# swook/EVE

Hardware: AMD Instinct MI355X
Metric: train-step frames/sec, 128x128 eye patches T=30 (higher is better)
Workload: dtype bf16; 1 GPU; BASELINE configs[1]: EyeNet training (configs/eye_net.json: ResNet-18-IN + GRU-128, angular + pupil L1 losses, clip 5.0, Adam wd 0.005), 128x128 patches, fwd+bwd+clip+Adam; global_batch=32, batch_per_gpu=32, seq_len=30, parallelism=dp1

## Files before the change

eve_amd/csrc/conv_igemm.hip:

```cpp
#include <limits.h>
#include <stdio.h>
#include <stdlib.h>

#include <initializer_list>
#include <type_traits>
#include "common.h"

namespace eve {

struct GatherParams {
    int N, IH, IW, Cin;
    int OH, OW, Cout;
    int KH, KW;
    int o_mul, k_mul, off, div;
    int K;
    uint32_t M;
    FastDiv fd_ohw, fd_ow, fd_cin, fd_kw, fd_oh;
};

template <typename T>
__device__ __forceinline__ uint4 prologue_vec(uint4 q, const float* __restrict__ ssp, int act) {
    constexpr int VEC = Elem<T>::VEC;
    float f[VEC];
    Elem<T>::unpack(q, f);
// ... 478 lines not shown
}

template <typename T>
static void launch_dma_one(const GatherParams& p, const TapPlan& tp, const void* src, const void* w,
                           const float* bias, int epi_act, void* out, uint32_t src_bytes, uint32_t w_bytes,
                           hipStream_t s) {
    const T* a = (const T*)src; const T* b = (const T*)w; T* o = (T*)out;
    const int big = g_cfg.conv_tile_big;
    if (p.Cout > 64 && big && p.M >= 256 * 256) {
        const uint32_t tiles = ((p.M + 255) / 256) * ((p.Cout + 127) / 128);
        EVE_LAUNCH("igemm_dma_kernel<T, 4, 2>", (igemm_dma_kernel<T, 4, 2>), dim3(tiles), dim3(512), 0, s, p, a, b, bias, epi_act, o,
                           src_bytes, w_bytes, tp);
    } else if (p.Cout > 64) {
        const uint32_t tiles = ((p.M + 127) / 128) * ((p.Cout + 127) / 128);
        EVE_LAUNCH("igemm_dma_kernel<T, 2, 2>", (igemm_dma_kernel<T, 2, 2>), dim3(tiles), dim3(256), 0, s, p, a, b, bias, epi_act, o,
                           src_bytes, w_bytes, tp);
    } else {
        const uint32_t tiles = (p.M + 255) / 256;
        EVE_LAUNCH("igemm_dma_kernel<T, 4, 1>", (igemm_dma_kernel<T, 4, 1>), dim3(tiles), dim3(256), 0, s, p, a, b, bias, epi_act, o,
                           src_bytes, w_bytes, tp);
    }
}

template <typename HT>
static bool launch_halo(const GatherParams& p, const void* src, const void* w, const float* bias, int epi_act,
                        void* out, hipStream_t s) {
    if (!g_cfg.conv_halo) return false;
    const bool fwd = p.k_mul == 1 && p.off == -1, bwd = p.k_mul == -1 && p.off == 1;
    if (p.KH != 3 || p.KW != 3 || p.div != 1 || p.o_mul != 1 || !(fwd || bwd) || p.OH != p.IH || p.OW != p.IW) return false;
    const int W = p.IW, H = p.IH;
    if (p.Cin % 32 || W > 128 || (W & (W - 1)) || W < 4) return false;
    HaloParams h;
    h.N = p.N; h.H = H; h.W = W; h.Cin = p.Cin; h.Cout = p.Cout;
    const int ws64 = g_cfg.conv_ws64;
    if (ws64 && H == W && (W == 32 || W == 64) && p.Cin == 64 && p.Cout == 64 && ((epi_act & ~0xff) == 0) &&
        ((epi_act & 0xff) == EVE_ACT_NONE || (epi_act & 0xff) == EVE_ACT_RELU) && (unsigned long long)p.N * W * W * 128ull < (1ull << 31)) {
        Ws64Params q;
        q.N = p.N; q.flip = bwd ? 1 : 0; q.x_bytes = (uint32_t)((unsigned long long)p.N * W * W * 128ull); q.w_bytes = 64u * 576u * 2u;
        const uint32_t T64 = (uint32_t)(W * W / 512) * (uint32_t)p.N;
        if (W == 32)
            launch(EVE_KERNEL_H(HT, conv3x3_ws64_kernel, 32), dim3(T64 < 256u ? T64 : 256u), dim3(512), (size_t)Ws64Geom<32>::LDS, s, q,
                   (const HT*)src, (const HT*)w, bias, epi_act, (HT*)out);
        else
            launch(EVE_KERNEL_H(HT, conv3x3_ws64_kernel, 64), dim3(T64 < 256u ? T64 : 256u), dim3(512), (size_t)Ws64Geom<64>::LDS, s, q,
                   (const HT*)src, (const HT*)w, bias, epi_act, (HT*)out);
        return true;
    }
    const int wg8 = g_cfg.conv_wg8;
    const int wg8_min_tiles = g_cfg.conv_wg8_min_tiles;
    if (wg8 && H == W && p.Cin % 64 == 0 && ((epi_act & ~0xff) == 0) &&
        ((epi_act & 0xff) == EVE_ACT_NONE || (epi_act & 0xff) == EVE_ACT_RELU)) {
        const unsigned long long xb8 = (unsigned long long)p.N * H * W * p.Cin * 2, wb8 = (unsigned long long)p.Cout * p.K * 2;
        Wg8Params g;
        g.N = p.N; g.Cin = p.Cin; g.Cout = p.Cout; g.flip = bwd ? 1 : 0; g.K = p.K; g.x_bytes = (uint32_t)xb8; g.w_bytes = (uint32_t)wb8; g.s2_py = 0;
        auto wg8_tile = [&](auto kernel, auto geom, uint32_t units) {
            using G8 = decltype(geom);
            g.tiles_n = (uint32_t)(p.Cout / G8::COUT_T);
            const uint32_t tiles8 = (units + G8::TI - 1) / G8::TI * g.tiles_n;
            if ((int)tiles8 < wg8_min_tiles) return false;
            launch(kernel, dim3(tiles8), dim3(512), G8::LDS, s, g, (const HT*)src, (const HT*)w, bias, epi_act, (HT*)out);
            return true;
        };
        const uint32_t imgs = (uint32_t)p.N;
        if (xb8 < (1ull << 31) && wb8 < (1ull << 31)) {
            if (wg8 != 3 && W == 16 && p.Cout % 128 == 0 && p.Cout % 256 != 0 &&
                wg8_tile(EVE_KERNEL_H(HT, conv3x3_wg8_kernel, 4, 2, 16), Wg8Geom<4, 2, 16>{}, imgs)) return true;
            if (W == 16 && p.Cout % 256 == 0 && wg8_tile(EVE_KERNEL_H(HT, conv3x3_wg8_kernel, 2, 4, 16), Wg8Geom<2, 4, 16>{}, imgs)) return true;
            if (W == 8 && p.Cout % 256 == 0 && wg8_tile(EVE_KERNEL_H(HT, conv3x3_wg8_kernel, 2, 4, 8), Wg8Geom<2, 4, 8>{}, imgs)) return true;
            if (W == 4 && p.Cout % 256 == 0 && wg8_tile(EVE_KERNEL_H(HT, conv3x3_wg8_kernel, 2, 4, 4), Wg8Geom<2, 4, 4>{}, imgs)) return true;
            if (W == 32 && p.Cout % 128 == 0 &&
                wg8_tile(EVE_KERNEL_H(HT, conv3x3_wg8_kernel, 4, 2, 32, 9, 2), Wg8Geom<4, 2, 32, 2>{}, 2u * imgs)) return true;
        }
    }
    const bool narrow = p.Cout <= 64;
    const int BMp = narrow ? 256 : 128;
    const int rows = BMp / W;
    if (rows < 1) return false;
    if (rows <= H) { h.TI = 1; h.TH = rows; h.bands = (H + rows - 1) / rows; }
    else { if (rows % H) return false; h.TI = rows / H; h.TH = H; h.bands = 1; }
    const int HP = h.TI * (h.TH + 2) * (W + 2);
    h.a_pieces = (HP * 4 + 255) / 256;
    if (h.a_pieces > 7) return false;
    const unsigned long long xb = (unsigned long long)p.N * H * W * p.Cin * 2, wb = (unsigned long long)p.Cout * p.K * 2;
    if (xb >= (1ull << 31) || wb >= (1ull << 31)) return false;
    h.flip = bwd ? 1 : 0; h.K = p.K; h.x_bytes = (uint32_t)xb; h.w_bytes = (uint32_t)wb;
    h.tiles_m = h.TI == 1 ? (uint32_t)p.N * h.bands : (uint32_t)((p.N + h.TI - 1) / h.TI);
    h.tiles_n = narrow ? 1 : (p.Cout + 127) / 128;
    h.fd_w2 = make_fastdiv(W + 2); h.fd_hpi = make_fastdiv((h.TH + 2) * (W + 2)); h.fd_w = make_fastdiv(W); h.fd_th = make_fastdiv(h.TH);
    const size_t lds = 2 * (size_t)h.a_pieces * 4096 + 4 * (narrow ? 4096 : 8192);
    const int persist = g_cfg.halo_persist;
    const uint32_t tiles = h.tiles_m * h.tiles_n;
    if (persist && tiles > 512 && p.Cin <= 64 && p.Cout % 8 == 0 && (epi_act == EVE_ACT_NONE || epi_act == EVE_ACT_RELU)) {
        const size_t plds = lds + (bias ? (size_t)h.tiles_n * (narrow ? 64 : 128) * 4 : 0);
        if (narrow)
            launch(EVE_KERNEL_H(HT, conv3x3_halo_pkernel, 4, 1), dim3(512), dim3(256), plds, s, h, (const HT*)src, (const HT*)w, bias, epi_act, (HT*)out);
        else
            launch(EVE_KERNEL_H(HT, conv3x3_halo_pkernel, 2, 2), dim3(512), dim3(256), plds, s, h, (const HT*)src, (const HT*)w, bias, epi_act, (HT*)out);
        return true;
    }
    if (narrow)
        launch(EVE_KERNEL_H(HT, conv3x3_halo_kernel, 4, 1), dim3(tiles), dim3(256), lds, s, h, (const HT*)src, (const HT*)w, bias, epi_act, (HT*)out);
    else
        launch(EVE_KERNEL_H(HT, conv3x3_halo_kernel, 2, 2), dim3(tiles), dim3(256), lds, s, h, (const HT*)src, (const HT*)w, bias, epi_act, (HT*)out);
    return true;
}

template <typename T>
// ... 216 lines not shown
                wgrad_split(p, tk, tc, lds_bytes(64, 256, mode), splits, rows);
                if (mode == 1)      tr_tile(EVE_WGRAD_TR(T, 1, 4, 1, 4), tk, tc);
                else if (mode == 2) {
                    if (p.Cout <= 16)      tr_tile(EVE_WGRAD_TR(T, 1, 4, 2, 1), tk, tc);
                    else if (p.Cout <= 32) tr_tile(EVE_WGRAD_TR(T, 1, 4, 2, 2), tk, tc);
                    else                   tr_tile(EVE_WGRAD_TR(T, 1, 4, 2, 4), tk, tc);
                }
                else                tr_tile(EVE_WGRAD_TR(T, 1, 4, 0, 4), tk, tc);
            }
            return db ? 1 : 0;
        }
    }
    }
    const bool wide = p.Cout > 64;
    const uint32_t bco = wide ? 128 : 64;
    const uint32_t tk = (p.K + 127) / 128, tc = (p.Cout + bco - 1) / bco;
    uint32_t want = (1024 + tk * tc - 1) / (tk * tc);
    uint32_t max_splits = (p.M + 255) / 256;
    uint32_t splits = want < 1 ? 1 : (want > max_splits ? max_splits : want);
    if (splits < 1) splits = 1;
    if (splits > 65535) splits = 65535;
    uint32_t rows = (p.M + splits - 1) / splits;
    rows = (rows + 63) / 64 * 64;
    splits = (p.M + rows - 1) / rows;
    dim3 grid(tk, tc, splits), block(256);
    const T* a = (const T*)x; const T* b = (const T*)dy;
    if (wide) {
        if (ss) EVE_LAUNCH("wgrad_kernel<T, 4, true>", (wgrad_kernel<T, 4, true>), grid, block, 0, s, p, a, b, ss, pro_act, dw, rows);
        else    EVE_LAUNCH("wgrad_kernel<T, 4, false>", (wgrad_kernel<T, 4, false>), grid, block, 0, s, p, a, b, ss, pro_act, dw, rows);
    } else {
        if (ss) EVE_LAUNCH("wgrad_kernel<T, 2, true>", (wgrad_kernel<T, 2, true>), grid, block, 0, s, p, a, b, ss, pro_act, dw, rows);
        else    EVE_LAUNCH("wgrad_kernel<T, 2, false>", (wgrad_kernel<T, 2, false>), grid, block, 0, s, p, a, b, ss, pro_act, dw, rows);
    }
    return 0;
}

template <typename HT>
static bool launch_s2_fwd_wg8(const eve_conv_desc* d, const void* x, const void* w, const float* bias, int epi_act, void* y, hipStream_t s) {
    const int on = g_cfg.conv_wg8, min_tiles = g_cfg.conv_wg8_s2_min_tiles;
    const int W = d->OW;
    if (!on || d->KH != 3 || d->KW != 3 || d->stride != 2 || d->pad != 1 || d->OH != W || d->IH != 2 * W || d->IW != 2 * W ||
        !(W == 16 || W == 8 || W == 4) || d->Cin % 64 || (epi_act & ~0xff) ||
        !((epi_act & 0xff) == EVE_ACT_NONE || (epi_act & 0xff) == EVE_ACT_RELU))
        return false;
    const int cout_t = W == 16 ? 128 : 256;
    if (d->Cout % cout_t) return false;
    const unsigned long long xb = (unsigned long long)d->N * 4 * W * W * d->Cin * 2, wb = (unsigned long long)d->Cout * 9 * d->Cin * 2;
    if (xb >= (1ull << 31) || wb >= (1ull << 31)) return false;
    const int ti = W == 16 ? 2 : (W == 8 ? 4 : 16);
    const uint32_t tiles = (uint32_t)((d->N + ti - 1) / ti) * (uint32_t)(d->Cout / cout_t);
    if ((int)tiles < min_tiles) return false;
    Wg8Params g;
    g.N = d->N; g.Cin = d->Cin; g.Cout = d->Cout; g.flip = 0; g.K = 9 * d->Cin; g.x_bytes = (uint32_t)xb; g.w_bytes = (uint32_t)wb;
    g.tiles_n = (uint32_t)(d->Cout / cout_t); g.s2_py = 0;
    auto s2_tile = [&](auto kernel, auto geom) {
        launch(kernel, dim3(tiles), dim3(512), decltype(geom)::LDS, s, g, (const HT*)x, (const HT*)w, bias, epi_act, (HT*)y);
    };
    if (W == 16) s2_tile(EVE_KERNEL_H(HT, conv3x3s2_wg8_kernel, 4, 2, 16), Wg8S2Geom<4, 2, 16>{});
    else if (W == 8) s2_tile(EVE_KERNEL_H(HT, conv3x3s2_wg8_kernel, 2, 4, 8), Wg8S2Geom<2, 4, 8>{});
    else s2_tile(EVE_KERNEL_H(HT, conv3x3s2_wg8_kernel, 2, 4, 4), Wg8S2Geom<2, 4, 4>{});
    return true;
}

template <typename H>
__global__ __launch_bounds__(256) void s2_dgrad_pack_kernel(const H* __restrict__ w_ihwo, H* __restrict__ w0, H* __restrict__ w1,
                                                            int Cdx, int Cout) {
    const int kv = Cout / 8;
    const long long n0 = (long long)2 * Cdx * 2 * kv, n1 = (long long)2 * Cdx * 4 * kv;
    for (long long i = (long long)blockIdx.x * 256 + threadIdx.x; i < n0 + n1; i += (long long)gridDim.x * 256) {
        const int py = i >= n0 ? 1 : 0, nt = py ? 4 : 2;
        const long long r = py ? i - n0 : i;
        const int v = (int)(r % kv), t = (int)((r / kv) % nt), row = (int)(r / ((long long)kv * nt));
        const int px = row >= Cdx ? 1 : 0, ci = row - px * Cdx;
        const int dy = py ? t >> 1 : 0, dx = t & 1;
        const int kh = py + 1 - 2 * dy, kw = px + 1 - 2 * dx;
        uint4 q = make_uint4(0u, 0u, 0u, 0u);
        if (kh >= 0 && kw >= 0)
            q = reinterpret_cast<const uint4*>(w_ihwo + (((size_t)ci * 3 + kh) * 3 + kw) * Cout)[v];
        reinterpret_cast<uint4*>(py ? w1 : w0)[r] = q;
    }
}

#define EVE_S2_DGRAD(H, WM, WN, W, NT) eve::Named<conv3x3_wg8_kernel<H, WM, WN, W, NT>>{EVE_HNAME(H, "conv3x3_wg8_kernel<", ", " #WM ", " #WN ", " #W ", s2dgrad" #NT ">")}, Wg8Geom<WM, WN, W>{}, ic<NT>{}

template <typename HT>
static bool launch_s2_dgrad_wg8(const eve_conv_desc* d, const void* dy, const void* w_ihwo, void* dx, void* workspace,
                                unsigned long long workspace_bytes, hipStream_t s) {
    const int on = g_cfg.conv_wg8, min_tiles = g_cfg.conv_wg8_s2_min_tiles;
    const int W = d->OW, Cdx = d->Cin, Co = d->Cout;
    if (!on || d->KH != 3 || d->KW != 3 || d->stride != 2 || d->pad != 1 || d->OH != W || d->IH != 2 * W || d->IW != 2 * W ||
        !(W == 16 || W == 8 || W == 4) || Co % 64 || !workspace || ((uintptr_t)workspace & 255))
        return false;
    const int cout_t = W == 16 ? 128 : 256;
    if ((2 * Cdx) % cout_t) return false;
    const unsigned long long wbytes = (unsigned long long)2 * Cdx * 6 * Co * 2;
    const unsigned long long xb = (unsigned long long)d->N * W * W * Co * 2, ob = (unsigned long long)d->N * 4 * W * W * Cdx * 2;
    if (wbytes > workspace_bytes || xb >= (1ull << 31) || ob >= (1ull << 31) || wbytes >= (1ull << 31)) return false;
    const int ti = W == 16 ? 2 : (W == 8 ? 4 : 16);
    const uint32_t tiles = (uint32_t)((d->N + ti - 1) / ti) * (uint32_t)(2 * Cdx / cout_t);
    if ((int)tiles < min_tiles) return false;
    HT* w0 = (HT*)workspace;
    HT* w1 = w0 + (size_t)2 * Cdx * 2 * Co;
    const long long nvec = (long long)2 * Cdx * 6 * (Co / 8);
    hipLaunchKernelGGL(s2_dgrad_pack_kernel<HT>, dim3((unsigned)((nvec + 255) / 256 > 1024 ? 1024 : (nvec + 255) / 256)), dim3(256), 0, s,
                       (const HT*)w_ihwo, w0, w1, Cdx, Co);
    Wg8Params g;
    g.N = d->N; g.Cin = Co; g.Cout = 2 * Cdx; g.flip = 0; g.x_bytes = (uint32_t)xb; g.tiles_n = (uint32_t)(2 * Cdx / cout_t);
    auto row_parity = [&](auto kernel, auto geom, auto nt, const HT* wp, int py) {
        constexpr int NT = decltype(nt)::value;
        g.K = NT * Co; g.w_bytes = (uint32_t)((unsigned long long)2 * Cdx * NT * Co * 2); g.s2_py = py;
        launch(kernel, dim3(tiles), dim3(512), decltype(geom)::LDS, s, g, (const HT*)dy, wp, (const float*)nullptr, (int)EVE_ACT_NONE, (HT*)dx);
    };
    if (W == 16) { row_parity(EVE_S2_DGRAD(HT, 4, 2, 16, 2), w0, 0); row_parity(EVE_S2_DGRAD(HT, 4, 2, 16, 4), w1, 1); }
    else if (W == 8) { row_parity(EVE_S2_DGRAD(HT, 2, 4, 8, 2), w0, 0); row_parity(EVE_S2_DGRAD(HT, 2, 4, 8, 4), w1, 1); }
    else { row_parity(EVE_S2_DGRAD(HT, 2, 4, 4, 2), w0, 0); row_parity(EVE_S2_DGRAD(HT, 2, 4, 4, 4), w1, 1); }
    return true;
}

static int conv_entry(const char* who, const eve_conv_desc* d, const char* cout_msg, bool operands, int max_cout_vecs = INT_MAX) {
    const int vec = (d && d->dtype != EVE_DT_F32) ? 8 : 4;
    if (int e = check_desc(d, vec)) return e;
    char msg[128];
    if (cout_msg && (d->Cout % vec || d->Cout / vec > max_cout_vecs)) { snprintf(msg, sizeof(msg), "%s: %s", who, cout_msg); return set_error_msg(msg); }
    if (!operands) { snprintf(msg, sizeof(msg), "%s: null pointer", who); return set_error_msg(msg); }
    return 0;
}

struct ConvCall {
    const char* who;
    const eve_conv_desc* d;
    bool dgrad;
    const void* in; const void* w; const float* bias; int epi_act; void* out;
    const float* in_scale_shift; int pro_act;
    void* workspace; unsigned long long workspace_bytes;
    hipStream_t s;
    int cin() const { return dgrad ? d->Cout : d->Cin; }
    int cout() const { return dgrad ? d->Cin : d->Cout; }
};
typedef bool (*ConvRung)(const ConvCall&);

static bool rung_1x1_stream(const ConvCall& c) {
    const eve_conv_desc* d = c.d;
    if (!(d->KH == 1 && d->KW == 1 && d->stride == 1 && d->pad == 0)) return false;
    const long long M = (long long)d->N * d->OH * d->OW;
    bool done = false;
    EVE_DISPATCH_H16(d->dtype, done = launch_conv1x1_stream<H>(M, c.cin(), c.cout(), c.in, c.w, c.bias, c.epi_act, c.out, c.s));
    return done;
}
static bool rung_1x1_s2_stream(const ConvCall& c) {
    const eve_conv_desc* d = c.d;
    if (!(!c.bias && c.epi_act == (c.dgrad ? (int)EVE_EPI_ACC : (int)EVE_ACT_NONE) && d->KH == 1 && d->stride == 2)) return false;
    bool done = false;
    EVE_DISPATCH_H16(d->dtype, done = launch_conv1x1_s2_stream<H>(d, c.dgrad, c.in, c.w, c.out, c.s));
    return done;
}
static bool rung_3x3_stream(const ConvCall& c) {
    const eve_conv_desc* d = c.d;
    if (!(d->KH == 3 && d->KW == 3 && d->stride == 1 && d->pad == 1)) return false;
    bool done = false;
    EVE_DISPATCH_H16(d->dtype, done = launch_conv3x3_stream<H>(d->N, d->IH, d->IW, c.cin(), c.cout(), c.dgrad ? 1 : 0, c.in, c.w, c.bias, c.epi_act,
                                                               c.out, c.s));
    return done;
}
static bool rung_s2_wg8(const ConvCall& c) {
    bool done = false;
    if (c.dgrad) EVE_DISPATCH_H16(c.d->dtype, done = launch_s2_dgrad_wg8<H>(c.d, c.in, c.w, c.out, c.workspace, c.workspace_bytes, c.s));
    else         EVE_DISPATCH_H16(c.d->dtype, done = launch_s2_fwd_wg8<H>(c.d, c.in, c.w, c.bias, c.epi_act, c.out, c.s));
    return done;
}
static int conv_ladder(const ConvCall& c, std::initializer_list<ConvRung> rungs) {
    bool done = false;
    if (!c.in_scale_shift && c.d->dtype != EVE_DT_F32)
        for (ConvRung rung : rungs)
            if ((done = rung(c))) break;
    if (!done) {
        const GatherParams p = c.dgrad ? dgrad_params(c.d) : fwd_params(c.d);
        EVE_DISPATCH_T(c.d->dtype, launch_igemm<T>(p, c.in, c.w, c.bias, c.in_scale_shift, c.pro_act, c.epi_act, c.out, c.s));
    }
    const hipError_t e = take_launch_error();
    return e == hipSuccess ? 0 : set_error(e, c.who);
}

}

using namespace eve;

extern "C" int eve_conv2d_fwd(const eve_conv_desc* d, const void* x, const void* w_ohwi, const float* bias,
                              int epi_act, const float* in_scale_shift, int pro_act, void* y,
                              eve_stream_t stream) {
    if (int e = conv_entry("conv2d_fwd", d, nullptr, x && w_ohwi && y)) return e;
    const ConvCall c = {__func__, d, false, x, w_ohwi, bias, epi_act, y, in_scale_shift, pro_act, nullptr, 0, (hipStream_t)stream};
    return conv_ladder(c, {rung_1x1_stream, rung_1x1_s2_stream, rung_3x3_stream, rung_s2_wg8});
}

extern "C" int eve_conv2d_fwd_stats(const eve_conv_desc* d, const void* x, const void* w_ohwi, const float* bias, int epi_act,
                                    void* y, float* mean_rstd, float eps, int* stats_written, eve_stream_t stream) {
    if (!stats_written || !mean_rstd) return set_error_msg("conv2d_fwd_stats: null pointer");
    *stats_written = 0;
    if (int e = conv_entry("conv2d_fwd_stats", d, nullptr, x && w_ohwi && y)) return e;
    if (d->KH == 3 && d->KW == 3 && d->stride == 1 && d->pad == 1 && d->dtype != EVE_DT_F32 && !(epi_act & EVE_EPI_ACC)) {
        bool done = false;
        EVE_DISPATCH_H16(d->dtype, done = launch_conv3x3_stream<H>(d->N, d->IH, d->IW, d->Cin, d->Cout, 0, x, w_ohwi, bias, epi_act, y,
                                                                   (hipStream_t)stream, mean_rstd, eps));
        if (done) { *stats_written = 1; EVE_CHECK_LAUNCH(); return 0; }
    }
    return eve_conv2d_fwd(d, x, w_ohwi, bias, epi_act, nullptr, 0, y, stream);
}

extern "C" int eve_conv2d_dgrad(const eve_conv_desc* d, const void* dy, const void* w_ihwo, void* dx,
                                void* workspace, unsigned long long workspace_bytes, eve_stream_t stream) {
    if (int e = conv_entry("conv2d_dgrad", d, "Cout must be a multiple of the 16-byte vector", dy && w_ihwo && dx)) return e;
    const ConvCall c = {__func__, d, true, dy, w_ihwo, nullptr, 0, dx, nullptr, 0, workspace, workspace_bytes, (hipStream_t)stream};
    return conv_ladder(c, {rung_1x1_stream, rung_3x3_stream, rung_s2_wg8});
}

extern "C" int eve_conv2d_dgrad_acc(const eve_conv_desc* d, const void* dy, const void* w_ihwo, void* dx,
                                    eve_stream_t stream) {
    if (int e = conv_entry("conv2d_dgrad_acc", d, "Cout must be a multiple of the 16-byte vector", dy && w_ihwo && dx)) return e;
    const ConvCall c = {__func__, d, true, dy, w_ihwo, nullptr, EVE_EPI_ACC, dx, nullptr, 0, nullptr, 0, (hipStream_t)stream};
// ... 77 lines not shown
```

eve_amd/csrc/conv_wg8.h:

```cpp
#pragma once
#include <type_traits>
#include "common.h"
#include "lds_dma.h"

namespace eve {

struct Wg8Params {
    int N, Cin, Cout;
    int flip;
    int K;
    uint32_t x_bytes, w_bytes;
    uint32_t tiles_n;
    int s2_py;
};

template <int W>
__device__ __forceinline__ int wg8_key(int hy, int hx) {
    return W >= 32 ? (hx >> 2) & 3 : (W >= 8 ? (hx >> 1) & 3 : hy & 3);
}
__device__ __forceinline__ int wg8_row_channel(int r64) {
    const int ct = r64 >> 5, i = r64 & 31;
    return 32 * ((i >> 2) & 1) + 16 * ct + 4 * (i >> 3) + (i & 3);
}

#define EVE_WG8_MMA_BODY(OP)                                                                                              \
    asm volatile(                                                                                                        \
        "s_nop 1\n\t"                                                                                                    \
        OP " %0, %8, %12, %0\n\t"  OP " %1, %8, %14, %1\n\t"  OP " %2, %8, %16, %2\n\t"  OP " %3, %8, %18, %3\n\t"          \
        OP " %4, %10, %12, %4\n\t" OP " %5, %10, %14, %5\n\t" OP " %6, %10, %16, %6\n\t" OP " %7, %10, %18, %7\n\t"        \
        OP " %0, %9, %13, %0\n\t"  OP " %1, %9, %15, %1\n\t"  OP " %2, %9, %17, %2\n\t"  OP " %3, %9, %19, %3\n\t"          \
        OP " %4, %11, %13, %4\n\t" OP " %5, %11, %15, %5\n\t" OP " %6, %11, %17, %6\n\t" OP " %7, %11, %19, %7"            \
        : "+a"(acc[0][0]), "+a"(acc[0][1]), "+a"(acc[0][2]), "+a"(acc[0][3]), "+a"(acc[1][0]), "+a"(acc[1][1]),          \
          "+a"(acc[1][2]), "+a"(acc[1][3])                                                                               \
        : "v"(wf[0][0]), "v"(wf[0][1]), "v"(wf[1][0]), "v"(wf[1][1]), "v"(xf[0][0]), "v"(xf[0][1]), "v"(xf[1][0]),        \
          "v"(xf[1][1]), "v"(xf[2][0]), "v"(xf[2][1]), "v"(xf[3][0]), "v"(xf[3][1]))
template <typename H>
__device__ __forceinline__ void wg8_mma16(f32x16_t (&acc)[2][4], const u32x4_t (&wf)[2][2], const u32x4_t (&xf)[4][2]) {
    if constexpr (Elem<H>::IS_BF16) { EVE_WG8_MMA_BODY("v_mfma_f32_32x32x16_bf16"); }
    else { EVE_WG8_MMA_BODY("v_mfma_f32_32x32x16_f16"); }
}
#undef EVE_WG8_MMA_BODY

template <int WM, int WN, int W, int BANDS = 1> struct Wg8Geom {
    static constexpr int PIX = 128 * WM, COUT_T = 64 * WN;
    static constexpr int TH = W / BANDS, UPIX = TH * W;
    static constexpr int TI = PIX / UPIX;
    static constexpr int W2 = W + 2, HPI = (TH + 2) * W2, HP = TI * HPI;
    static constexpr int APT = (HP + 15) / 16;
    static constexpr int AP = (APT + 7) / 8;
    static constexpr int ASTAGE = AP * 8 * 1024;
    static constexpr int BSLOT = COUT_T * 64;
    static constexpr int BP = COUT_T / 16 / 8;
    static constexpr int LDS = 2 * ASTAGE + 4 * BSLOT;
    static_assert(WM * WN == 8 && W % BANDS == 0 && PIX % UPIX == 0 && TI >= 1 && (BANDS == 1 || TI == 1) && AP <= 7 && BP >= 1 &&
                  LDS <= 160 * 1024, "tile geometry");
};

template <typename H, int WM, int WN, int W, int NT = 9, int BANDS = 1>
__global__ __launch_bounds__(512, 2) void conv3x3_wg8_kernel(const Wg8Params p, const H* __restrict__ x,
                                                             const H* __restrict__ w, const float* __restrict__ bias,
                                                             const int epi_act, H* __restrict__ out) {
    using G = Wg8Geom<WM, WN, W, BANDS>;
    static_assert(BANDS == 1 || (NT == 9 && W >= 8), "row bands: the 3x3 convolution on W >= 8");
    constexpr int W2 = G::W2, HPI = G::HPI, HP = G::HP, AP = G::AP, BP = G::BP, ASTAGE = G::ASTAGE, BSLOT = G::BSLOT;
    constexpr int TH = G::TH, UPIX = G::UPIX;
    extern __shared__ __attribute__((aligned(16))) char smem[];

    const int tid = threadIdx.x;
    const int wave = __builtin_amdgcn_readfirstlane(tid >> 6);
    const int lane = tid & 63;
    const uint32_t lid = xcd_remap(blockIdx.x, gridDim.x);
    const uint32_t tm = lid / p.tiles_n, tn = lid - tm * p.tiles_n;
    const uint32_t n0 = tm * G::TI, co0 = tn * G::COUT_T;

    const eve_int4 rs_x = make_rsrc_words(x, p.x_bytes);
    const eve_int4 rs_w = make_rsrc_words(w, p.w_bytes);
    const uint32_t ldsA = lds_addr_of(smem), ldsB = ldsA + 2 * ASTAGE;

    int a_goff[AP];
#pragma unroll
    for (int j = 0; j < AP; ++j) {
        const int hp = (j * 8 + wave) * 16 + (lane >> 2), pc = lane & 3;
        int off = EVE_OOB;
        if (hp < HP) {
            const int ti = hp / HPI, r = hp - ti * HPI, hy = r / W2, hx = r - hy * W2;
            const uint32_t u = n0 + ti, n = u / BANDS;
            const int gy = (int)(u % BANDS) * TH + hy - 1, gx = hx - 1;
            if (gy >= 0 && gy < W && gx >= 0 && gx < W && n < (uint32_t)p.N)
                off = (int)((((n * W + gy) * W + gx) * p.Cin) * 2) + ((pc ^ wg8_key<W>(hy, hx)) << 4);
        }
        a_goff[j] = off;
    }
    int b_goff[BP];
#pragma unroll
    for (int j = 0; j < BP; ++j) {
        const int row = (j * 8 + wave) * 16 + (lane >> 2), pc = lane & 3;
        const uint32_t co = co0 + (row & ~63) + wg8_row_channel(row & 63);
        b_goff[j] = co < (uint32_t)p.Cout ? (int)(co * (uint32_t)p.K) * 2 + ((pc ^ ((row >> 2) & 3)) << 4) : EVE_OOB;
    }

    const int wm = wave / WN, wn = wave - wm * WN;
    const int l31 = lane & 31, l5 = lane >> 5;
    uint32_t wrd[2][2];
#pragma unroll
    for (int ct = 0; ct < 2; ++ct)
#pragma unroll
        for (int kh = 0; kh < 2; ++kh) {
            const int row = wn * 64 + ct * 32 + l31;
            wrd[ct][kh] = ldsB + row * 64 + (((2 * kh + l5) ^ ((row >> 2) & 3)) << 4);
        }
    uint32_t xrd[4][3][2];
#pragma unroll
    for (int pt = 0; pt < 4; ++pt) {
        const int m = wm * 128 + pt * 32 + l31;
        const int ti = m / UPIX, ty = (m / W) % TH, tx = m % W;
#pragma unroll
        for (int q = 0; q < 3; ++q) {
            const int hy = W >= 8 ? ty : ty + q, hx = W >= 8 ? tx + q : tx;
#pragma unroll
            for (int kh = 0; kh < 2; ++kh)
                xrd[pt][q][kh] = ldsA + (ti * HPI + hy * W2 + hx) * 64 + (((2 * kh + l5) ^ wg8_key<W>(hy, hx)) << 4);
        }
    }

    f32x16_t acc[2][4];
#pragma unroll
    for (int a = 0; a < 2; ++a)
#pragma unroll
        for (int b = 0; b < 4; ++b)
#pragma unroll
            for (int r = 0; r < 16; ++r) acc[a][b][r] = 0.f;

    const int nslices = p.Cin / 32;
    const int cin2 = p.Cin * 2;
    const int tap_base = (NT == 9 && p.flip) ? 8 * cin2 : 0, tap_step = (NT == 9 && p.flip) ? -cin2 : cin2;
    auto issue_b = [&](int s, int t, int slot) {
        const int soff = tap_base + t * tap_step + s * 64;
#pragma unroll
        for (int j = 0; j < BP; ++j) lds_dma16_asm(rs_w, ldsB + slot * BSLOT + (j * 8 + wave) * 1024, b_goff[j], soff);
    };

#pragma unroll
    for (int j = 0; j < AP; ++j) lds_dma16_asm(rs_x, ldsA + (j * 8 + wave) * 1024, a_goff[j], 0);
    issue_b(0, 0, 0);
    issue_b(0, 1, 1);
    wait_vm<0>();
    __builtin_amdgcn_s_barrier();

    const bool lead = wave < 4;
    u32x4_t wf[2][2], xf[4][2];
#pragma unroll
    for (int i = 0; i < 2; ++i)
#pragma unroll
        for (int j = 0; j < 2; ++j) wf[i][j] = u32x4_t{0u, 0u, 0u, 0u};
#pragma unroll
    for (int i = 0; i < 4; ++i)
#pragma unroll
        for (int j = 0; j < 2; ++j) xf[i][j] = u32x4_t{0u, 0u, 0u, 0u};
    if (!lead) __builtin_amdgcn_s_setprio(2);

    for (int s2 = 0; s2 < nslices; s2 += 2) {
#pragma unroll
        for (int ss = 0; ss < 2; ++ss) {
            const int s = s2 + ss;
            const bool last = s + 1 == nslices;
#pragma unroll
            for (int t = 0; t < NT; ++t) {
                const int dy = NT == 9 ? t / 3 : (NT == 4 ? 1 + t / 2 : 1), dx = NT == 9 ? t % 3 : 1 + (t & 1);
                const int t2 = (t + 2) % NT, sd = (t + 2) / NT;
                const bool more_b = !(last && sd);
                constexpr int PPS = NT == 9 ? 1 : (AP + NT - 2) / (NT - 1);
                const int j0 = NT == 9 ? t - 1 : t * PPS;
                const int np = NT == 9 ? ((t >= 1 && t <= AP) ? 1 : 0) : (j0 >= AP ? 0 : (j0 + PPS <= AP ? PPS : AP - j0));
                if (!lead) wg8_mma16<H>(acc, wf, xf);
                const uint32_t slot_off = (uint32_t)((NT * s + t) & 3) * BSLOT;
#pragma unroll
                for (int ct = 0; ct < 2; ++ct)
#pragma unroll
                    for (int kh = 0; kh < 2; ++kh)
                        wf[ct][kh] = lds_read16(wrd[ct][kh] + slot_off);
                const int imm = ss * ASTAGE + (W >= 8 ? dy * W2 * 64 : dx * 64);
                const int q = W >= 8 ? dx : dy;
#pragma unroll
                for (int pt = 0; pt < 4; ++pt)
#pragma unroll
                    for (int kh = 0; kh < 2; ++kh)
                        xf[pt][kh] = lds_read16(xrd[pt][q][kh] + imm);
                if (more_b) issue_b(s + sd, t2, (NT * s + t + 2) & 3);
                if (!last) {
#pragma unroll
                    for (int jj = 0; jj < PPS; ++jj)
                        if (jj < np) lds_dma16_asm(rs_x, ldsA + (ss ^ 1) * ASTAGE + ((j0 + jj) * 8 + wave) * 1024, a_goff[jj < np ? j0 + jj : 0], (s + 1) * 64);
                }
                if (lead) wg8_mma16<H>(acc, wf, xf);
                if (more_b) {
                    if (!last) {
                        if (np == 0) wait_vm<BP>();
                        else if (np == 1) wait_vm<BP + 1>();
                        else if (np == 2) wait_vm<BP + 2>();
                        else if (np == 3) wait_vm<BP + 3>();
                        else if (np == 4) wait_vm<BP + 4>();
                        else if (np == 5) wait_vm<BP + 5>();
                        else wait_vm<BP + 6>();
                    } else wait_vm<BP>();
                } else {
                    wait_vm<0>();
                }
                __builtin_amdgcn_s_barrier();
            }
        }
    }
    if (!lead) wg8_mma16<H>(acc, wf, xf);
    __builtin_amdgcn_s_setprio(0);
    asm volatile("s_nop 15\n\ts_nop 15"
                 : "+a"(acc[0][0]), "+a"(acc[0][1]), "+a"(acc[0][2]), "+a"(acc[0][3]), "+a"(acc[1][0]), "+a"(acc[1][1]),
                   "+a"(acc[1][2]), "+a"(acc[1][3]) :: "memory");

    const uint32_t co = co0 + wn * 64 + l5 * 32;
    const bool relu = (epi_act & 0xff) == EVE_ACT_RELU;
    float bv[32];
#pragma unroll
    for (int c = 0; c < 32; c += 4) {
        const float4 b4 = bias ? *reinterpret_cast<const float4*>(bias + co + c) : make_float4(0.f, 0.f, 0.f, 0.f);
        bv[c] = b4.x; bv[c + 1] = b4.y; bv[c + 2] = b4.z; bv[c + 3] = b4.w;
    }
#pragma unroll
    for (int pt = 0; pt < 4; ++pt) {
        __builtin_amdgcn_sched_barrier(0);
        const int m = wm * 128 + pt * 32 + l31;
        const int ti = m / UPIX;
        const uint32_t u = n0 + ti, n = u / BANDS;
        const int pix = m - ti * UPIX + (int)(u % BANDS) * UPIX;
        u32x4_t pk[4];
#pragma unroll
        for (int ct = 0; ct < 2; ++ct)
#pragma unroll
            for (int r = 0; r < 16; r += 2) {
                float o0 = acc[ct][pt][r] + bv[ct * 16 + r], o1 = acc[ct][pt][r + 1] + bv[ct * 16 + r + 1];
                if (relu) { o0 = fmaxf(o0, 0.f); o1 = fmaxf(o1, 0.f); }
                pk[ct * 2 + (r >> 3)][(r >> 1) & 3] = Elem<H>::pack2(o0, o1);
            }
        quad_transpose4x4(pk, lane);
        if (n < (uint32_t)p.N) {
            if constexpr (NT == 9) {
                H* dst = out + ((size_t)n * (W * W) + (pix & ~3)) * p.Cout + co + (l31 & 3) * 8;
#pragma unroll
                for (int v = 0; v < 4; ++v) *reinterpret_cast<u32x4_t*>(dst + (size_t)v * p.Cout) = pk[v];
            } else {
                const int cdx = p.Cout >> 1, px = (int)co >= cdx ? 1 : 0, ci = (int)co - px * cdx;
                const int pb = pix & ~3, yy = pb / W, xx = pb - yy * W;
                H* dst = out + (((size_t)n * (2 * W) + 2 * yy + p.s2_py) * (2 * W) + 2 * xx + px) * cdx + ci + (l31 & 3) * 8;
#pragma unroll
                for (int v = 0; v < 4; ++v) *reinterpret_cast<u32x4_t*>(dst + (size_t)(2 * v) * cdx) = pk[v];
            }
        }
    }
}

}
```

Before: 91660 frames/s.

## Fuse stride-2 dgrad parity classes into one launch and skip zero-weight taps

Replaces the stride-2 data-gradient path, which packed weights into a workspace and then ran two kernel launches (one per row parity), with a single launch. Each block derives its row and column parity class from its tile id and reads the original weights directly. Each class issues only the taps whose weights are nonzero: 1, 2, 2 or 4. The centre class takes a dedicated compact path that streams only the unpadded input through three LDS stages. This removes the pack kernel, one launch and the work spent multiplying padded zero taps. In exchange the kernel gains more template variants, code size and register pressure, and blocks now carry unequal amounts of work.

```diff
diff --git a/eve_amd/csrc/conv_igemm.hip b/eve_amd/csrc/conv_igemm.hip
--- a/eve_amd/csrc/conv_igemm.hip
+++ b/eve_amd/csrc/conv_igemm.hip
@@ -554,7 +554,7 @@
         ((epi_act & 0xff) == EVE_ACT_NONE || (epi_act & 0xff) == EVE_ACT_RELU)) {
         const unsigned long long xb8 = (unsigned long long)p.N * H * W * p.Cin * 2, wb8 = (unsigned long long)p.Cout * p.K * 2;
         Wg8Params g;
-        g.N = p.N; g.Cin = p.Cin; g.Cout = p.Cout; g.flip = bwd ? 1 : 0; g.K = p.K; g.x_bytes = (uint32_t)xb8; g.w_bytes = (uint32_t)wb8; g.s2_py = 0;
+        g.N = p.N; g.Cin = p.Cin; g.Cout = p.Cout; g.flip = bwd ? 1 : 0; g.K = p.K; g.x_bytes = (uint32_t)xb8; g.w_bytes = (uint32_t)wb8;
         auto wg8_tile = [&](auto kernel, auto geom, uint32_t units) {
             using G8 = decltype(geom);
             g.tiles_n = (uint32_t)(p.Cout / G8::COUT_T);
@@ -877,7 +877,7 @@
     if ((int)tiles < min_tiles) return false;
     Wg8Params g;
     g.N = d->N; g.Cin = d->Cin; g.Cout = d->Cout; g.flip = 0; g.K = 9 * d->Cin; g.x_bytes = (uint32_t)xb; g.w_bytes = (uint32_t)wb;
-    g.tiles_n = (uint32_t)(d->Cout / cout_t); g.s2_py = 0;
+    g.tiles_n = (uint32_t)(d->Cout / cout_t);
     auto s2_tile = [&](auto kernel, auto geom) {
         launch(kernel, dim3(tiles), dim3(512), decltype(geom)::LDS, s, g, (const HT*)x, (const HT*)w, bias, epi_act, (HT*)y);
     };
@@ -887,58 +887,33 @@
     return true;
 }
 
-template <typename H>
-__global__ __launch_bounds__(256) void s2_dgrad_pack_kernel(const H* __restrict__ w_ihwo, H* __restrict__ w0, H* __restrict__ w1,
-                                                            int Cdx, int Cout) {
-    const int kv = Cout / 8;
-    const long long n0 = (long long)2 * Cdx * 2 * kv, n1 = (long long)2 * Cdx * 4 * kv;
-    for (long long i = (long long)blockIdx.x * 256 + threadIdx.x; i < n0 + n1; i += (long long)gridDim.x * 256) {
-        const int py = i >= n0 ? 1 : 0, nt = py ? 4 : 2;
-        const long long r = py ? i - n0 : i;
-        const int v = (int)(r % kv), t = (int)((r / kv) % nt), row = (int)(r / ((long long)kv * nt));
-        const int px = row >= Cdx ? 1 : 0, ci = row - px * Cdx;
-        const int dy = py ? t >> 1 : 0, dx = t & 1;
-        const int kh = py + 1 - 2 * dy, kw = px + 1 - 2 * dx;
-        uint4 q = make_uint4(0u, 0u, 0u, 0u);
-        if (kh >= 0 && kw >= 0)
-            q = reinterpret_cast<const uint4*>(w_ihwo + (((size_t)ci * 3 + kh) * 3 + kw) * Cout)[v];
-        reinterpret_cast<uint4*>(py ? w1 : w0)[r] = q;
-    }
-}
-
-#define EVE_S2_DGRAD(H, WM, WN, W, NT) eve::Named<conv3x3_wg8_kernel<H, WM, WN, W, NT>>{EVE_HNAME(H, "conv3x3_wg8_kernel<", ", " #WM ", " #WN ", " #W ", s2dgrad" #NT ">")}, Wg8Geom<WM, WN, W>{}, ic<NT>{}
+#define EVE_S2_DGRAD(H, NWM, NWN, WM, WN, W) eve::Named<conv3x3_wg8_kernel<H, WM, WN, W, 4>>{EVE_HNAME(H, "conv3x3_wg8_kernel<", ", " #NWM ", " #NWN ", " #W ", s2dgrad4>")}, Wg8Geom<WM, WN, W>{}
 
 template <typename HT>
-static bool launch_s2_dgrad_wg8(const eve_conv_desc* d, const void* dy, const void* w_ihwo, void* dx, void* workspace,
-                                unsigned long long workspace_bytes, hipStream_t s) {
+static bool launch_s2_dgrad_wg8(const eve_conv_desc* d, const void* dy, const void* w_ihwo, void* dx, hipStream_t s) {
     const int on = g_cfg.conv_wg8, min_tiles = g_cfg.conv_wg8_s2_min_tiles;
     const int W = d->OW, Cdx = d->Cin, Co = d->Cout;
     if (!on || d->KH != 3 || d->KW != 3 || d->stride != 2 || d->pad != 1 || d->OH != W || d->IH != 2 * W || d->IW != 2 * W ||
-        !(W == 16 || W == 8 || W == 4) || Co % 64 || !workspace || ((uintptr_t)workspace & 255))
+        !(W == 16 || W == 8 || W == 4) || Co % 64)
         return false;
-    const int cout_t = W == 16 ? 128 : 256;
-    if ((2 * Cdx) % cout_t) return false;
-    const unsigned long long wbytes = (unsigned long long)2 * Cdx * 6 * Co * 2;
+    const int floor_cout_t = W == 16 ? 128 : 256;
+    if ((2 * Cdx) % floor_cout_t) return false;
+    const unsigned long long wbytes = (unsigned long long)Cdx * 9 * Co * 2;
     const unsigned long long xb = (unsigned long long)d->N * W * W * Co * 2, ob = (unsigned long long)d->N * 4 * W * W * Cdx * 2;
-    if (wbytes > workspace_bytes || xb >= (1ull << 31) || ob >= (1ull << 31) || wbytes >= (1ull << 31)) return false;
-    const int ti = W == 16 ? 2 : (W == 8 ? 4 : 16);
-    const uint32_t tiles = (uint32_t)((d->N + ti - 1) / ti) * (uint32_t)(2 * Cdx / cout_t);
-    if ((int)tiles < min_tiles) return false;
-    HT* w0 = (HT*)workspace;
-    HT* w1 = w0 + (size_t)2 * Cdx * 2 * Co;
-    const long long nvec = (long long)2 * Cdx * 6 * (Co / 8);
-    hipLaunchKernelGGL(s2_dgrad_pack_kernel<HT>, dim3((unsigned)((nvec + 255) / 256 > 1024 ? 1024 : (nvec + 255) / 256)), dim3(256), 0, s,
-                       (const HT*)w_ihwo, w0, w1, Cdx, Co);
+    if (xb >= (1ull << 31) || ob >= (1ull << 31) || wbytes >= (1ull << 31)) return false;
+    const int floor_ti = W == 16 ? 2 : (W == 8 ? 4 : 16);
+    if ((int)((uint32_t)((d->N + floor_ti - 1) / floor_ti) * (uint32_t)(2 * Cdx / floor_cout_t)) < min_tiles) return false;
     Wg8Params g;
-    g.N = d->N; g.Cin = Co; g.Cout = 2 * Cdx; g.flip = 0; g.x_bytes = (uint32_t)xb; g.tiles_n = (uint32_t)(2 * Cdx / cout_t);
-    auto row_parity = [&](auto kernel, auto geom, auto nt, const HT* wp, int py) {
-        constexpr int NT = decltype(nt)::value;
-        g.K = NT * Co; g.w_bytes = (uint32_t)((unsigned long long)2 * Cdx * NT * Co * 2); g.s2_py = py;
-        launch(kernel, dim3(tiles), dim3(512), decltype(geom)::LDS, s, g, (const HT*)dy, wp, (const float*)nullptr, (int)EVE_ACT_NONE, (HT*)dx);
+    g.N = d->N; g.Cin = Co; g.Cout = 2 * Cdx; g.flip = 0; g.K = 9 * Co; g.x_bytes = (uint32_t)xb; g.w_bytes = (uint32_t)wbytes;
+    auto classes = [&](auto kernel, auto geom) {
+        using G8 = decltype(geom);
+        g.tiles_n = (uint32_t)(2 * Cdx / G8::COUT_T);
+        const uint32_t tiles = (uint32_t)((d->N + G8::TI - 1) / G8::TI) * 2u * g.tiles_n;
+        launch(kernel, dim3(tiles), dim3(512), G8::LDS, s, g, (const HT*)dy, (const HT*)w_ihwo, (const float*)nullptr, (int)EVE_ACT_NONE, (HT*)dx);
     };
-    if (W == 16) { row_parity(EVE_S2_DGRAD(HT, 4, 2, 16, 2), w0, 0); row_parity(EVE_S2_DGRAD(HT, 4, 2, 16, 4), w1, 1); }
-    else if (W == 8) { row_parity(EVE_S2_DGRAD(HT, 2, 4, 8, 2), w0, 0); row_parity(EVE_S2_DGRAD(HT, 2, 4, 8, 4), w1, 1); }
-    else { row_parity(EVE_S2_DGRAD(HT, 2, 4, 4, 2), w0, 0); row_parity(EVE_S2_DGRAD(HT, 2, 4, 4, 4), w1, 1); }
+    if (W == 16) classes(EVE_S2_DGRAD(HT, 4, 2, 4, 2, 16));
+    else if (W == 8) classes(EVE_S2_DGRAD(HT, 2, 4, 4, 2, 8));
+    else classes(EVE_S2_DGRAD(HT, 2, 4, 2, 4, 4));
     return true;
 }
 
@@ -989,7 +964,7 @@
 }
 static bool rung_s2_wg8(const ConvCall& c) {
     bool done = false;
-    if (c.dgrad) EVE_DISPATCH_H16(c.d->dtype, done = launch_s2_dgrad_wg8<H>(c.d, c.in, c.w, c.out, c.workspace, c.workspace_bytes, c.s));
+    if (c.dgrad) EVE_DISPATCH_H16(c.d->dtype, done = launch_s2_dgrad_wg8<H>(c.d, c.in, c.w, c.out, c.s));
     else         EVE_DISPATCH_H16(c.d->dtype, done = launch_s2_fwd_wg8<H>(c.d, c.in, c.w, c.bias, c.epi_act, c.out, c.s));
     return done;
 }
diff --git a/eve_amd/csrc/conv_wg8.h b/eve_amd/csrc/conv_wg8.h
--- a/eve_amd/csrc/conv_wg8.h
+++ b/eve_amd/csrc/conv_wg8.h
@@ -11,7 +11,6 @@
     int K;
     uint32_t x_bytes, w_bytes;
     uint32_t tiles_n;
-    int s2_py;
 };
 
 template <int W>
@@ -61,7 +60,9 @@
                                                              const H* __restrict__ w, const float* __restrict__ bias,
                                                              const int epi_act, H* __restrict__ out) {
     using G = Wg8Geom<WM, WN, W, BANDS>;
+    static_assert(NT == 9 || NT == 4, "the 3x3 convolution or the stride-2 data gradient");
     static_assert(BANDS == 1 || (NT == 9 && W >= 8), "row bands: the 3x3 convolution on W >= 8");
+    constexpr bool S2 = NT != 9;
     constexpr int W2 = G::W2, HPI = G::HPI, HP = G::HP, AP = G::AP, BP = G::BP, ASTAGE = G::ASTAGE, BSLOT = G::BSLOT;
     constexpr int TH = G::TH, UPIX = G::UPIX;
     extern __shared__ __attribute__((aligned(16))) char smem[];
@@ -70,12 +71,24 @@
     const int wave = __builtin_amdgcn_readfirstlane(tid >> 6);
     const int lane = tid & 63;
     const uint32_t lid = xcd_remap(blockIdx.x, gridDim.x);
-    const uint32_t tm = lid / p.tiles_n, tn = lid - tm * p.tiles_n;
+    uint32_t tm, tn;
+    int py = 0;
+    if constexpr (S2) {
+        const uint32_t grp = 2 * p.tiles_n;
+        tm = lid / grp;
+        const uint32_t r = lid - tm * grp;
+        py = r < p.tiles_n ? 1 : 0;
+        tn = p.tiles_n - 1 - (py ? r : r - p.tiles_n);
+    } else {
+        tm = lid / p.tiles_n; tn = lid - tm * p.tiles_n;
+    }
     const uint32_t n0 = tm * G::TI, co0 = tn * G::COUT_T;
 
     const eve_int4 rs_x = make_rsrc_words(x, p.x_bytes);
     const eve_int4 rs_w = make_rsrc_words(w, p.w_bytes);
     const uint32_t ldsA = lds_addr_of(smem), ldsB = ldsA + 2 * ASTAGE;
+    const int nslices = p.Cin / 32;
+    const int cin2 = p.Cin * 2;
 
     int a_goff[AP];
 #pragma unroll
@@ -91,12 +104,20 @@
         }
         a_goff[j] = off;
     }
-    int b_goff[BP];
+    int b_goff[BP], b_goff1[S2 ? BP : 1];
 #pragma unroll
     for (int j = 0; j < BP; ++j) {
         const int row = (j * 8 + wave) * 16 + (lane >> 2), pc = lane & 3;
         const uint32_t co = co0 + (row & ~63) + wg8_row_channel(row & 63);
-        b_goff[j] = co < (uint32_t)p.Cout ? (int)(co * (uint32_t)p.K) * 2 + ((pc ^ ((row >> 2) & 3)) << 4) : EVE_OOB;
+        const int chunk = (pc ^ ((row >> 2) & 3)) << 4;
+        if constexpr (S2) {
+            const uint32_t cdx = (uint32_t)p.Cout >> 1, px = co >= cdx ? 1u : 0u, ci = co - px * cdx;
+            const int base = (int)(ci * (uint32_t)p.K) * 2 + chunk;
+            b_goff[j] = co < (uint32_t)p.Cout ? base + (px ? cin2 : 0) : EVE_OOB;
+            b_goff1[j] = (co < (uint32_t)p.Cout && px) ? base : EVE_OOB;
+        } else {
+            b_goff[j] = co < (uint32_t)p.Cout ? (int)(co * (uint32_t)p.K) * 2 + chunk : EVE_OOB;
+        }
     }
 
     const int wm = wave / WN, wn = wave - wm * WN;
@@ -109,19 +130,6 @@
             const int row = wn * 64 + ct * 32 + l31;
             wrd[ct][kh] = ldsB + row * 64 + (((2 * kh + l5) ^ ((row >> 2) & 3)) << 4);
         }
-    uint32_t xrd[4][3][2];
-#pragma unroll
-    for (int pt = 0; pt < 4; ++pt) {
-        const int m = wm * 128 + pt * 32 + l31;
-        const int ti = m / UPIX, ty = (m / W) % TH, tx = m % W;
-#pragma unroll
-        for (int q = 0; q < 3; ++q) {
-            const int hy = W >= 8 ? ty : ty + q, hx = W >= 8 ? tx + q : tx;
-#pragma unroll
-            for (int kh = 0; kh < 2; ++kh)
-                xrd[pt][q][kh] = ldsA + (ti * HPI + hy * W2 + hx) * 64 + (((2 * kh + l5) ^ wg8_key<W>(hy, hx)) << 4);
-        }
-    }
 
     f32x16_t acc[2][4];
 #pragma unroll
@@ -130,22 +138,6 @@
         for (int b = 0; b < 4; ++b)
 #pragma unroll
             for (int r = 0; r < 16; ++r) acc[a][b][r] = 0.f;
-
-    const int nslices = p.Cin / 32;
-    const int cin2 = p.Cin * 2;
-    const int tap_base = (NT == 9 && p.flip) ? 8 * cin2 : 0, tap_step = (NT == 9 && p.flip) ? -cin2 : cin2;
-    auto issue_b = [&](int s, int t, int slot) {
-        const int soff = tap_base + t * tap_step + s * 64;
-#pragma unroll
-        for (int j = 0; j < BP; ++j) lds_dma16_asm(rs_w, ldsB + slot * BSLOT + (j * 8 + wave) * 1024, b_goff[j], soff);
-    };
-
-#pragma unroll
-    for (int j = 0; j < AP; ++j) lds_dma16_asm(rs_x, ldsA + (j * 8 + wave) * 1024, a_goff[j], 0);
-    issue_b(0, 0, 0);
-    issue_b(0, 1, 1);
-    wait_vm<0>();
-    __builtin_amdgcn_s_barrier();
 
     const bool lead = wave < 4;
     u32x4_t wf[2][2], xf[4][2];
@@ -157,58 +149,163 @@
     for (int i = 0; i < 4; ++i)
 #pragma unroll
         for (int j = 0; j < 2; ++j) xf[i][j] = u32x4_t{0u, 0u, 0u, 0u};
-    if (!lead) __builtin_amdgcn_s_setprio(2);
-
-    for (int s2 = 0; s2 < nslices; s2 += 2) {
-#pragma unroll
-        for (int ss = 0; ss < 2; ++ss) {
-            const int s = s2 + ss;
-            const bool last = s + 1 == nslices;
-#pragma unroll
-            for (int t = 0; t < NT; ++t) {
-                const int dy = NT == 9 ? t / 3 : (NT == 4 ? 1 + t / 2 : 1), dx = NT == 9 ? t % 3 : 1 + (t & 1);
-                const int t2 = (t + 2) % NT, sd = (t + 2) / NT;
-                const bool more_b = !(last && sd);
-                constexpr int PPS = NT == 9 ? 1 : (AP + NT - 2) / (NT - 1);
-                const int j0 = NT == 9 ? t - 1 : t * PPS;
-                const int np = NT == 9 ? ((t >= 1 && t <= AP) ? 1 : 0) : (j0 >= AP ? 0 : (j0 + PPS <= AP ? PPS : AP - j0));
-                if (!lead) wg8_mma16<H>(acc, wf, xf);
-                const uint32_t slot_off = (uint32_t)((NT * s + t) & 3) * BSLOT;
-#pragma unroll
-                for (int ct = 0; ct < 2; ++ct)
-#pragma unroll
-                    for (int kh = 0; kh < 2; ++kh)
-                        wf[ct][kh] = lds_read16(wrd[ct][kh] + slot_off);
-                const int imm = ss * ASTAGE + (W >= 8 ? dy * W2 * 64 : dx * 64);
-                const int q = W >= 8 ? dx : dy;
-#pragma unroll
-                for (int pt = 0; pt < 4; ++pt)
-#pragma unroll
-                    for (int kh = 0; kh < 2; ++kh)
-                        xf[pt][kh] = lds_read16(xrd[pt][q][kh] + imm);
-                if (more_b) issue_b(s + sd, t2, (NT * s + t + 2) & 3);
-                if (!last) {
-#pragma unroll
-                    for (int jj = 0; jj < PPS; ++jj)
-                        if (jj < np) lds_dma16_asm(rs_x, ldsA + (ss ^ 1) * ASTAGE + ((j0 + jj) * 8 + wave) * 1024, a_goff[jj < np ? j0 + jj : 0], (s + 1) * 64);
+
+    auto run = [&](auto ntb_c, auto vert_c, auto py_c) __attribute__((always_inline)) {
+        constexpr int NTB = decltype(ntb_c)::value, PY = decltype(py_c)::value;
+        constexpr bool VERT = decltype(vert_c)::value != 0;
+        uint32_t xrd[4][3][2];
+#pragma unroll
+        for (int pt = 0; pt < 4; ++pt) {
+            const int m = wm * 128 + pt * 32 + l31;
+            const int ti = m / UPIX, ty = (m / W) % TH, tx = m % W;
+#pragma unroll
+            for (int q = 0; q < 3; ++q) {
+                const int hy = W >= 8 ? ty : ty + q, hx = W >= 8 ? tx + q : tx;
+#pragma unroll
+                for (int kh = 0; kh < 2; ++kh)
+                    xrd[pt][q][kh] = ldsA + (ti * HPI + hy * W2 + hx) * 64 + (((2 * kh + l5) ^ wg8_key<W>(hy, hx)) << 4);
+            }
+        }
+        const int tap_base = p.flip ? 8 * cin2 : 0, tap_step = p.flip ? -cin2 : cin2;
+        auto issue_b = [&](int s, int t, int slot) {
+            if constexpr (NTB == 9) {
+                const int soff = tap_base + t * tap_step + s * 64;
+#pragma unroll
+                for (int j = 0; j < BP; ++j) lds_dma16_asm(rs_w, ldsB + slot * BSLOT + (j * 8 + wave) * 1024, b_goff[j], soff);
+            } else {
+                const int wdy = NTB == 4 ? t / 2 : (VERT ? t : 0), wdx = NTB == 4 ? t & 1 : (VERT ? 0 : t);
+                const int soff = ((PY + 1 - 2 * wdy) * 3 + (wdx ? 0 : 1)) * cin2 + s * 64;
+#pragma unroll
+                for (int j = 0; j < BP; ++j)
+                    lds_dma16_asm(rs_w, ldsB + slot * BSLOT + (j * 8 + wave) * 1024, wdx ? b_goff1[j] : b_goff[j], soff);
+            }
+        };
+
+#pragma unroll
+        for (int j = 0; j < AP; ++j) lds_dma16_asm(rs_x, ldsA + (j * 8 + wave) * 1024, a_goff[j], 0);
+        issue_b(0, 0, 0);
+        issue_b(0, 1, 1);
+        wait_vm<0>();
+        __builtin_amdgcn_s_barrier();
+        if (!lead) __builtin_amdgcn_s_setprio(2);
+
+        for (int s2 = 0; s2 < nslices; s2 += 2) {
+#pragma unroll
+            for (int ss = 0; ss < 2; ++ss) {
+                const int s = s2 + ss;
+                const bool last = s + 1 == nslices;
+#pragma unroll
+                for (int t = 0; t < NTB; ++t) {
+                    const int dy = NTB == 9 ? t / 3 : 1 + (NTB == 4 ? t / 2 : (VERT ? t : 0));
+                    const int dx = NTB == 9 ? t % 3 : 1 + (NTB == 4 ? (t & 1) : (VERT ? 0 : t));
+                    const int t2 = (t + 2) % NTB, sd = (t + 2) / NTB;
+                    const bool more_b = !(last && sd);
+                    constexpr int PPS = NTB == 9 ? 1 : (AP + NTB - 2) / (NTB - 1);
+                    const int j0 = NTB == 9 ? t - 1 : t * PPS;
+                    const int np = NTB == 9 ? ((t >= 1 && t <= AP) ? 1 : 0) : (j0 >= AP ? 0 : (j0 + PPS <= AP ? PPS : AP - j0));
+                    if (!lead) wg8_mma16<H>(acc, wf, xf);
+                    const uint32_t slot_off = (uint32_t)((NTB * s + t) & 3) * BSLOT;
+#pragma unroll
+                    for (int ct = 0; ct < 2; ++ct)
+#pragma unroll
+                        for (int kh = 0; kh < 2; ++kh)
+                            wf[ct][kh] = lds_read16(wrd[ct][kh] + slot_off);
+                    const int imm = ss * ASTAGE + (W >= 8 ? dy * W2 * 64 : dx * 64);
+                    const int q = W >= 8 ? dx : dy;
+#pragma unroll
+                    for (int pt = 0; pt < 4; ++pt)
+#pragma unroll
+                        for (int kh = 0; kh < 2; ++kh)
+                            xf[pt][kh] = lds_read16(xrd[pt][q][kh] + imm);
+                    if (more_b) issue_b(s + sd, t2, (NTB * s + t + 2) & 3);
+                    if (!last) {
+#pragma unroll
+                        for (int jj = 0; jj < PPS; ++jj)
+                            if (jj < np) lds_dma16_asm(rs_x, ldsA + (ss ^ 1) * ASTAGE + ((j0 + jj) * 8 + wave) * 1024, a_goff[jj < np ? j0 + jj : 0], (s + 1) * 64);
+                    }
+                    if (lead) wg8_mma16<H>(acc, wf, xf);
+                    if (more_b) {
+                        if (!last) {
+                            if (np == 0) wait_vm<BP>();
+                            else if (np == 1) wait_vm<BP + 1>();
+                            else if (np == 2) wait_vm<BP + 2>();
+                            else if (np == 3) wait_vm<BP + 3>();
+                            else if (np == 4) wait_vm<BP + 4>();
+                            else if (np == 5) wait_vm<BP + 5>();
+                            else if (np == 6) wait_vm<BP + 6>();
+                            else wait_vm<BP + 7>();
+                        } else wait_vm<BP>();
+                    } else {
+                        wait_vm<0>();
+                    }
+                    __builtin_amdgcn_s_barrier();
                 }
-                if (lead) wg8_mma16<H>(acc, wf, xf);
-                if (more_b) {
-                    if (!last) {
-                        if (np == 0) wait_vm<BP>();
-                        else if (np == 1) wait_vm<BP + 1>();
-                        else if (np == 2) wait_vm<BP + 2>();
-                        else if (np == 3) wait_vm<BP + 3>();
-                        else if (np == 4) wait_vm<BP + 4>();
-                        else if (np == 5) wait_vm<BP + 5>();
-                        else wait_vm<BP + 6>();
-                    } else wait_vm<BP>();
-                } else {
-                    wait_vm<0>();
-                }
-                __builtin_amdgcn_s_barrier();
-            }
-        }
+            }
+        }
+    };
+
+    auto run_centre = [&]() __attribute__((always_inline)) {
+        constexpr int CP = G::PIX / 128, CSTAGE = G::PIX * 64;
+        static_assert(!S2 || 3 * CSTAGE <= 2 * ASTAGE, "three compact stages");
+        int c_goff[CP];
+        uint32_t c_lds[CP];
+#pragma unroll
+        for (int j = 0; j < CP; ++j) {
+            const int m = (j * 8 + wave) * 16 + (lane >> 2), pc = lane & 3;
+            const uint32_t n = n0 + m / UPIX;
+            c_goff[j] = n < (uint32_t)p.N ? (int)(((n0 * UPIX + m) * (uint32_t)p.Cin) * 2) + ((pc ^ ((m >> 2) & 3)) << 4) : EVE_OOB;
+            c_lds[j] = ldsA + (j * 8 + wave) * 1024;
+        }
+        uint32_t crd[4][2];
+#pragma unroll
+        for (int pt = 0; pt < 4; ++pt)
+#pragma unroll
+            for (int kh = 0; kh < 2; ++kh) {
+                const int m = wm * 128 + pt * 32 + l31;
+                crd[pt][kh] = ldsA + m * 64 + (((2 * kh + l5) ^ ((m >> 2) & 3)) << 4);
+            }
+        auto issue = [&](int s, uint32_t stage_off, int slot) {
+            const int soff = 4 * cin2 + s * 64;
+#pragma unroll
+            for (int j = 0; j < BP; ++j) lds_dma16_asm(rs_w, ldsB + slot * BSLOT + (j * 8 + wave) * 1024, b_goff[j], soff);
+#pragma unroll
+            for (int j = 0; j < CP; ++j) lds_dma16_asm(rs_x, c_lds[j] + stage_off, c_goff[j], s * 64);
+        };
+        issue(0, 0u, 0);
+        issue(1, (uint32_t)CSTAGE, 1);
+        wait_vm<0>();
+        __builtin_amdgcn_s_barrier();
+        if (!lead) __builtin_amdgcn_s_setprio(2);
+        uint32_t st = 0u, st2 = 2u * CSTAGE;
+        for (int s = 0; s < nslices; ++s) {
+            const bool more = s + 2 < nslices;
+            if (!lead) wg8_mma16<H>(acc, wf, xf);
+            const uint32_t slot_off = (uint32_t)(s & 3) * BSLOT;
+#pragma unroll
+            for (int ct = 0; ct < 2; ++ct)
+#pragma unroll
+                for (int kh = 0; kh < 2; ++kh)
+                    wf[ct][kh] = lds_read16(wrd[ct][kh] + slot_off);
+#pragma unroll
+            for (int pt = 0; pt < 4; ++pt)
+#pragma unroll
+                for (int kh = 0; kh < 2; ++kh)
+                    xf[pt][kh] = lds_read16(crd[pt][kh] + st);
+            if (more) issue(s + 2, st2, (s + 2) & 3);
+            if (lead) wg8_mma16<H>(acc, wf, xf);
+            if (more) wait_vm<BP + CP>(); else wait_vm<0>();
+            __builtin_amdgcn_s_barrier();
+            st = st == 2u * CSTAGE ? 0u : st + CSTAGE;
+            st2 = st2 == 2u * CSTAGE ? 0u : st2 + CSTAGE;
+        }
+    };
+
+    if constexpr (S2) {
+        const bool px0 = co0 + G::COUT_T <= ((uint32_t)p.Cout >> 1);
+        if (py) { if (px0) run(ic<2>{}, ic<1>{}, ic<1>{}); else run(ic<4>{}, ic<0>{}, ic<1>{}); }
+        else    { if (px0) run_centre();                   else run(ic<2>{}, ic<0>{}, ic<0>{}); }
+    } else {
+        run(ic<9>{}, ic<0>{}, ic<0>{});
     }
     if (!lead) wg8_mma16<H>(acc, wf, xf);
     __builtin_amdgcn_s_setprio(0);
@@ -249,7 +346,7 @@
             } else {
                 const int cdx = p.Cout >> 1, px = (int)co >= cdx ? 1 : 0, ci = (int)co - px * cdx;
                 const int pb = pix & ~3, yy = pb / W, xx = pb - yy * W;
-                H* dst = out + (((size_t)n * (2 * W) + 2 * yy + p.s2_py) * (2 * W) + 2 * xx + px) * cdx + ci + (l31 & 3) * 8;
+                H* dst = out + (((size_t)n * (2 * W) + 2 * yy + py) * (2 * W) + 2 * xx + px) * cdx + ci + (l31 & 3) * 8;
 #pragma unroll
                 for (int v = 0; v < 4; ++v) *reinterpret_cast<u32x4_t*>(dst + (size_t)(2 * v) * cdx) = pk[v];
             }
```

Result: slower. 90530 frames/s (-1.2%).
